# flanglet/kanzi-cpp

Measured on AMD Instinct MI355X. Metric: encode+decode MB/s on the synthetic stand-in for silesia.tar (bit-exact), higher is better.
Workload: dtype u8

## Files before the change

### kanzi-cpp_amd/csrc/bwt_fwd.hip

```cpp
#include "common.hpp"
#include "stages.hpp"
#include "bwt_common.hpp"

#include <cstdlib>
#include <cstring>
#include <algorithm>
#include <cmath>
#include "prims.hpp"
#include <chrono>
#include <vector>

namespace knz {

constexpr u32 SM_TS = 1792;
constexpr u32 SM_WIN = 2048;
constexpr u32 SM_G = 256;
constexpr u32 MED_CAP = 8192;
constexpr u32 SUPER_CAP = 8192;
constexpr int GATHER_THREADS = 512;
constexpr u32 GATHER_ROWS = 16;
static_assert(MED_CAP <= GATHER_ROWS * GATHER_THREADS, "k_bwt_f_gather_desc judges a medium group from one batch of loads");
constexpr u32 LARGE_OS_MIN = 1000000;
constexpr u32 NO_BIT = 0x7FFFFFFFu;

struct FwdView {
    const u32* base;
    int nBlocks;
    u32 total;
    u32* SA;
    u32* ISA;
    u64* ISA2;
    u32 round;
    u32* K;
    u32* gbits;
    u32* gnew;
    u32* counters;
    const u32* ovr;
    const u32* rtbits;
    uint2* medStage;
};

enum FwdCounter : u32 {
    CNT_SMALL_LEFT = 0,
    CNT_MED = 1,
    CNT_LARGE = 2,
    CNT_LARGE_MEMBERS = 3,
    CNT_RUN = 4,
    CNT_RUN_MEMBERS = 5,
    CNT_RUN_LONGEST = 6,
    CNT_SUPER = 7,
    CNT_RUNS = 8,
    CNT_STAT_SMALL = 10,
    CNT_STAT_SMALL_GROUPS = 11,
    CNT_STAT_MED = 12,
    CNT_TIED = 13,
    CNT_PROBE_CAND = 14,
    CNT_LINKED = 14,
    CNT_LINK_TIED = 15,
    CNT_STAT_MED_GROUPS = 16,
    CNT_STAT_UNSPLIT = 17,
    CNT_STAT_UNSPLIT_MEMBERS = 18,
    CNT_STAT_MAJ = 19,
    CNT_STAT_MAJ_MEMBERS = 20,
    CNT_ROUND_SLOTS = 24,
    CNT_PROBE_SLOTS = 2,
    CNT_LONGEST_BLOCK = 32,
    CNT_NSYM = 33,
};

constexpr u32 LAB_BITS = 28;
constexpr u64 LAB_MASK = (1ull << LAB_BITS) - 1ull;

__device__ __forceinline__ u32 lab_old(const FwdView& v, u32 q, u32 bb)
{
    if (v.ISA2 == nullptr) return v.ISA[q];
    const u64 e = v.ISA2[q];
    const u32 rel = ((u32)(e >> 56) == v.round && v.round != 0) ? (u32)((e >> LAB_BITS) & LAB_MASK) : (u32)(e & LAB_MASK);
    return bb + rel;
}
__device__ __forceinline__ u32 lab_cur(const FwdView& v, u32 q, u32 bb)
{
    if (v.ISA2 == nullptr) return v.ISA[q];
    return bb + (u32)(v.ISA2[q] & LAB_MASK);
}
__device__ __forceinline__ void lab_set(const FwdView& v, u32 p, u32 bb, u32 lab, u32 was)
{
    if (v.ISA2 == nullptr) { v.ISA[p] = lab; return; }
#ifdef KNZ_EMU
    if (v.round != 0 && lab_old(v, p, bb) != was) {
        fprintf(stderr, "lab_set: round %u position %u: was %u, label %u\n", v.round, p, was, lab_old(v, p, bb));
        abort();
    }
#endif
    const u64 nw = (u64)(lab - bb), ow = (v.round == 0) ? nw : (u64)(was - bb);
    v.ISA2[p] = nw | (ow << LAB_BITS) | ((u64)v.round << 56);
}

__device__ __forceinline__ u32 gather_key(const FwdView& v, u32 gp, u32 h, u32 blkBase, u32 blkEnd)
{
    const u32 q = gp + h;
    return (q < blkEnd) ? lab_old(v, q, blkBase) - blkBase + 1u : 0u;
}

__device__ __forceinline__ void classify_child(const FwdView& v, uint2* __restrict__ medNext, uint2* __restrict__ largeNext, u32 start, u32 size, u32& surv)
{
    if (size > MED_CAP) {
        const u32 at = atomicAdd(&v.counters[CNT_LARGE], 1u);
        largeNext[at] = make_uint2(start, size);
        atomicAdd(&v.counters[CNT_LARGE_MEMBERS], size);
    } else if (size > SM_G) {
        v.medStage[start >> 8] = make_uint2(start, size);
    } else if (size > 1) {
        surv = 1;
    }
}

struct ClassAgg { u32 cnt[3]; u32 elems[3]; u32 base[3]; };

__device__ __forceinline__ void agg_init(ClassAgg& A) { if (threadIdx.x < 3) { A.cnt[threadIdx.x] = 0; A.elems[threadIdx.x] = 0; A.base[threadIdx.x] = 0; } }

__device__ __forceinline__ int agg_note(ClassAgg& A, u32 size, bool run, u32& surv, u32& local)
{
    int kind;
    if (run) kind = 2;
    else if (size > MED_CAP) kind = 1;
    else if (size > SM_G) kind = 0;
    else { if (size > 1) surv = 1; return -1; }
    if (kind != 0) { local = atomicAdd(&A.cnt[kind], 1u); atomicAdd(&A.elems[kind], size); }
    return kind;
}

__device__ __forceinline__ void agg_reserve(ClassAgg& A, const FwdView& v)
{
    if (A.cnt[1]) { A.base[1] = atomicAdd(&v.counters[CNT_LARGE], A.cnt[1]); atomicAdd(&v.counters[CNT_LARGE_MEMBERS], A.elems[1]); }
    if (A.cnt[2]) { A.base[2] = atomicAdd(&v.counters[CNT_RUN], A.cnt[2]); atomicAdd(&v.counters[CNT_RUN_MEMBERS], A.elems[2]); }
}

__device__ __forceinline__ void agg_write(const ClassAgg& A, const FwdView& v, int kind, u32 local, u32 start, u32 size, uint2* __restrict__ largeNext,
                                          uint2* __restrict__ runList)
{
    if (kind == 0) { v.medStage[start >> 8] = make_uint2(start, size); return; }
    uint2* dst = kind == 1 ? largeNext : runList;
    dst[A.base[kind] + local] = make_uint2(start, size);
}

__global__ void k_bwt_bases(BwtView v, u32* __restrict__ base, u8* __restrict__ ok, u32* __restrict__ maxLen, int suffixOnly)
// ... 674 lines not shown
}

__device__ __forceinline__ u32 link_next_zero(const u32* __restrict__ posflag, const u32* __restrict__ sufRev, u32 nW, u32 p)
{
    const u32 w = p >> 5;
    const u32 x = ~posflag[w] & (0xFFFFFFFFu << (p & 31));
    if (x) return 32u * w + (u32)__ffs((int)x) - 1u;
    return (w + 1 < nW) ? sufRev[nW - 2 - w] : 0xFFFFFFFFu;
}

__global__ __launch_bounds__(256) void k_bwt_f_link_apply(FwdView v, const u32* __restrict__ posflag, const u32* __restrict__ sufRev, u32 nW,
                                                          const u32* __restrict__ linked, u32 h, u32* __restrict__ ovr, u32* __restrict__ rtbits, u32 tileStep, LinkTrial tr)
{
    __shared__ SmWindow W;
    __shared__ int sAny;
    __shared__ u32 sLinked[64];
    __shared__ u32 sRt[64];
    __shared__ u32 sOff[SM_WIN];
    u32 tile, posLo, posHi;
    if (!link_tile(v, tr, tileStep, tile, posLo, posHi)) return;
    const u32 slot0 = tile * SM_TS;
    if (threadIdx.x >= 64 && threadIdx.x < 128) { sLinked[threadIdx.x - 64] = linked[(slot0 >> 5) + threadIdx.x - 64]; sRt[threadIdx.x - 64] = 0; }
    if (!sm_load_window(v, slot0, W, &sAny)) return;
    __syncthreads();
    u32 gs[SM_WIN / 256], ge[SM_WIN / 256];
    bool act[SM_WIN / 256];
#pragma unroll
    for (int k = 0; k < (int)(SM_WIN / 256); k++) {
        const u32 i = threadIdx.x + 256u * k;
        act[k] = sm_group_of(W, i, gs[k], ge[k]) && ((sLinked[gs[k] >> 5] >> (gs[k] & 31)) & 1u);
        if (act[k] && i == gs[k]) {
            const u32 gp = v.SA[slot0 + i];
            const u32 e = link_next_zero(posflag, sufRev, nW, gp);
            sOff[i] = (e != 0xFFFFFFFFu && e > gp) ? (e - gp) + h : 0u;
        }
    }
    __syncthreads();
#pragma unroll
    for (int k = 0; k < (int)(SM_WIN / 256); k++) {
        if (!act[k]) continue;
        const u32 i = threadIdx.x + 256u * k;
        const u32 off = sOff[gs[k]];
        if (off == 0) continue;
        const u32 slot = slot0 + i;
        const bool had = (rtbits[slot >> 5] >> (slot & 31)) & 1u;
        const u32 old = had ? ovr[slot] : 0u;
        if (off > old) ovr[slot] = off;
        if (!had) atomicOr(&sRt[i >> 5], 1u << (i & 31));
    }
    __syncthreads();
    if (threadIdx.x < 64 && sRt[threadIdx.x]) atomicOr(&rtbits[(slot0 >> 5) + threadIdx.x], sRt[threadIdx.x]);
}

template <int ROWS>
__device__ __forceinline__ bool gather_rows(const FwdView& v, u32 gs, u32 n, u32 off, u32 bb, u32 be, bool judge, u32 key0, u32* sDiff)
{
    u32 gp[ROWS], key[ROWS];
#pragma unroll
    for (int k = 0; k < ROWS; k++) { const u32 i = (u32)k * GATHER_THREADS + threadIdx.x; gp[k] = (i < n) ? v.SA[gs + i] : bb; }
#pragma unroll
    for (int k = 0; k < ROWS; k++) { const u32 i = (u32)k * GATHER_THREADS + threadIdx.x; key[k] = (i < n) ? gather_key(v, gp[k], off, bb, be) : key0; }
    if (judge) {
        bool diff = false;
#pragma unroll
        for (int k = 0; k < ROWS; k++) diff = diff || key[k] != key0;
        if (__ballot(diff) != 0 && (threadIdx.x & 63) == 0) *sDiff = 1;
        __syncthreads();
        if (*sDiff == 0) return true;
    }
#pragma unroll
    for (int k = 0; k < ROWS; k++) { const u32 i = (u32)k * GATHER_THREADS + threadIdx.x; if (i < n) v.K[gs + i] = key[k]; }
    return false;
}

__global__ __launch_bounds__(GATHER_THREADS) void k_bwt_f_gather_desc(FwdView v, uint2* __restrict__ desc, u32 nDesc, u32 h, uint2* __restrict__ descInfo, int stats, int skip)
{
    __shared__ int sBlk;
    __shared__ u32 sDiff;
    const u32 xcd = blockIdx.x & 7, lanesPerXcd = gridDim.x >> 3, slot = blockIdx.x >> 3;
    const u32 per = (nDesc + 7) / 8;
    const u32 lo = xcd * per, hi = (lo + per < nDesc) ? lo + per : nDesc;
    for (u32 g = lo + slot; g < hi; g += lanesPerXcd) {
        const uint2 d = desc[g];
        if (threadIdx.x == 0) { sBlk = find_block(v.base, v.nBlocks, d.x); sDiff = 0; }
        __syncthreads();
        const u32 bb = v.base[sBlk], be = v.base[sBlk + 1];
        u32 off = h;
        if (v.rtbits && ((v.rtbits[d.x >> 5] >> (d.x & 31)) & 1u)) { const u32 r = v.ovr[d.x]; off = r > h ? r : h; }
        const u32 gp0 = v.SA[d.x];
        const u32 lab = lab_old(v, gp0, bb), key0 = gather_key(v, gp0, off, bb, be);
        const bool judge = skip && d.y > SM_G && d.y <= GATHER_ROWS * (u32)GATHER_THREADS && lab - d.x < d.y;
        bool unsplit = false;
        if (d.y <= 1 * GATHER_THREADS) unsplit = gather_rows<1>(v, d.x, d.y, off, bb, be, judge, key0, &sDiff);
        else if (d.y <= 2 * GATHER_THREADS) unsplit = gather_rows<2>(v, d.x, d.y, off, bb, be, judge, key0, &sDiff);
        else if (d.y <= 4 * GATHER_THREADS) unsplit = gather_rows<4>(v, d.x, d.y, off, bb, be, judge, key0, &sDiff);
        else if (d.y <= 8 * GATHER_THREADS) unsplit = gather_rows<8>(v, d.x, d.y, off, bb, be, judge, key0, &sDiff);
        else for (u32 i0 = 0; i0 < d.y; i0 += GATHER_ROWS * GATHER_THREADS)
            unsplit = gather_rows<(int)GATHER_ROWS>(v, d.x + i0, d.y - i0, off, bb, be, judge, key0, &sDiff);
        if (threadIdx.x == 0) {
            descInfo[g] = make_uint2(bb, lab);
            if (unsplit) { v.medStage[d.x >> 8] = d; desc[g] = make_uint2(d.x, 0u); }
            if (stats && d.y) {
                atomicAdd(&v.counters[CNT_STAT_MED], d.y); atomicAdd(&v.counters[CNT_STAT_MED_GROUPS], 1u);
                if (unsplit) { atomicAdd(&v.counters[CNT_STAT_UNSPLIT], 1u); atomicAdd(&v.counters[CNT_STAT_UNSPLIT_MEMBERS], d.y); }
            }
        }
        __syncthreads();
    }
}

template <int THREADS, int ROWS>
struct MedLds {
    static constexpr int WAVES = THREADS / 64;
    static constexpr u32 CAP = (u32)ROWS * THREADS;
    u32 oK[CAP];
    u32 oV[CAP];
    u32 cnt[WAVES * 256];
    u32 fb[CAP / 32];
    int pm[CAP / 32];
    u32 pn[CAP / 32];
    u32 wtot[WAVES];
    u32 wtot2[WAVES];
    u32 oldLab;
    u32 blkBase;
};

template <int THREADS, int ROWS>
__device__ __forceinline__ u32 med_block_sum(MedLds<THREADS, ROWS>& L, u32 x)
{
    const u32 s = wave_sum(x);
    if ((threadIdx.x & 63) == 0) L.wtot[threadIdx.x >> 6] = s;
    __syncthreads();
    u32 tot = 0;
    for (int w = 0; w < THREADS / 64; w++) tot += L.wtot[w];
    __syncthreads();
    return tot;
}

template <int THREADS, int ROWS>
__device__ __forceinline__ void med_radix_sort(MedLds<THREADS, ROWS>& L, u32 n, int npass)
{
    constexpr int WAVES = THREADS / 64;
    const int tid = (int)threadIdx.x, lane = tid & 63, wave = tid >> 6;
    const unsigned long long ltMask = (lane == 0) ? 0ull : (~0ull >> (64 - lane));
    u32* cntw = L.cnt + wave * 256;
    const int R = (int)((n + THREADS - 1) / THREADS);
    const u32 waveBase = (u32)wave * (u32)R * 64u;
    for (int pass = 0; pass < npass; pass++) {
        const int shift = 8 * pass;
        for (int q = lane; q < 256; q += 64) cntw[q] = 0;
        u32 key[ROWS], val[ROWS], pre[ROWS];
#pragma unroll
        for (int r = 0; r < ROWS; r++) {
            key[r] = 0xFFFFFFFFu; val[r] = 0; pre[r] = 0;
            if (r < R) {
                const u32 idx = waveBase + (u32)r * 64u + (u32)lane;
                if (idx < n) { key[r] = L.oK[idx]; val[r] = L.oV[idx]; }
                const u32 dg = (key[r] >> shift) & 255u;
                const unsigned long long peers = prims::digit_peers_fast(true, dg);
                const u32 pop = (u32)__popcll(peers);
                const u32 rnk = (u32)__popcll(peers & ltMask);
                const int leader = __ffsll((long long)peers) - 1;
                u32 old = 0;
                if (lane == leader) { old = cntw[dg]; cntw[dg] = old + pop; }
                old = (u32)__shfl((int)old, leader, 64);
                pre[r] = old + rnk;
            }
        }
        __syncthreads();
        {
            constexpr int TPD = THREADS / 256;
            const int dg = tid / TPD, w0 = (tid % TPD) * 4;
            const u32 c0 = L.cnt[(w0 + 0) * 256 + dg], c1 = L.cnt[(w0 + 1) * 256 + dg], c2 = L.cnt[(w0 + 2) * 256 + dg], c3 = L.cnt[(w0 + 3) * 256 + dg];
            const u32 sum = c0 + c1 + c2 + c3;
            const u32 incl = wave_incl_scan(sum);
            if (lane == 63) L.wtot[wave] = incl;
            __syncthreads();
            u32 wbase = 0;
            for (int w = 0; w < wave; w++) wbase += L.wtot[w];
            const u32 excl = wbase + incl - sum;
            L.cnt[(w0 + 0) * 256 + dg] = excl;
            L.cnt[(w0 + 1) * 256 + dg] = excl + c0;
            L.cnt[(w0 + 2) * 256 + dg] = excl + c0 + c1;
            L.cnt[(w0 + 3) * 256 + dg] = excl + c0 + c1 + c2;
        }
        __syncthreads();
#pragma unroll
        for (int r = 0; r < ROWS; r++) {
            if (r < R) {
                const u32 dg = (key[r] >> shift) & 255u;
// ... 882 lines not shown
        for (int which = 0; which < 2; which++) {
            const unsigned long long mask = which ? rm : hm;
            u32* dst = which ? rtbits : v.gnew;
            if (mask == 0) continue;
            const u32 p0 = (u32)(mask << sh);
            const u32 p1 = sh ? (u32)(mask >> (32 - sh)) : (u32)(mask >> 32);
            const u32 p2 = sh ? (u32)(mask >> (64 - sh)) : 0u;
            if (p0) atomicOr(&dst[w0], p0);
            if (p1) atomicOr(&dst[w0 + 1], p1);
            if (p2) atomicOr(&dst[w0 + 2], p2);
        }
    }
}

__global__ __launch_bounds__(256) void k_bwt_f_merge_bits(u32* __restrict__ gbits, u32* __restrict__ gnew, u32 nWords)
{
    const u32 w = blockIdx.x * 256 + threadIdx.x;
    if (w >= nWords) return;
    const u32 x = gnew[w];
    if (x) { gbits[w] |= x; gnew[w] = 0; }
}

__global__ __launch_bounds__(256) void k_bwt_f_emit(BwtView v, const u32* __restrict__ base, const u8* __restrict__ ok, const u32* __restrict__ SA,
                                                    FwdView fv, u32* __restrict__ newLen)
{
    const int b = blockIdx.y;
    if (!ok[b]) return;
    const u32 n = v.len[b];
    u32 pIndexSize = 0;
    bwt_fwd_applies(n, v.cap[b], &pIndexSize);
    const int chunks = bwt_chunks(n);
    const u32 hdr = 1 + (u32)chunks * pIndexSize;
    const u8* s = v.src[b];
    u8* d = v.dst[b];
    const u32 bb = base[b];
    const u32 r0 = lab_cur(fv, bb, bb) - bb;
    const u32 qLo = hdr + 1, qHi = hdr + n;
    const bool al = (reinterpret_cast<uintptr_t>(d) & 3) == 0;
    for (u32 w = (qLo >> 2) + blockIdx.x * 256 + threadIdx.x; 4 * w < qHi; w += gridDim.x * 256) {
        u32 word = 0, have = 0;
#pragma unroll
        for (u32 k = 0; k < 4; k++) {
            const u32 q = 4 * w + k;
            if (q >= qLo && q < qHi) {
                const u32 rr = q - qLo;
                const u32 r = rr + (rr >= r0 ? 1u : 0u);
                const u32 p = SA[bb + r] - bb;
                word |= (u32)s[p - 1] << (8 * k);
                have |= 1u << k;
            }
        }
        if (have == 0xF && al) reinterpret_cast<u32*>(d)[w] = word;
        else for (u32 k = 0; k < 4; k++) if ((have >> k) & 1) d[4 * w + k] = (u8)(word >> (8 * k));
    }
    if (blockIdx.x == 0 && threadIdx.x == 0) {
        d[hdr] = s[n - 1];
        const u32 st = n / (u32)chunks;
        const u32 step = ((u32)chunks * st == n) ? st : st + 1;
        const u32 logNbChunks = (u32)ilog2_u32((u32)chunks);
        d[0] = (u8)((logNbChunks << 2) | (pIndexSize - 1));
        u32 idx = 1;
        for (int k = 0; k < chunks; k++) {
            const u32 prim = lab_cur(fv, bb + (u32)k * step, bb) - bb;
            for (int sh = (int)(pIndexSize - 1) * 8; sh >= 0; sh -= 8) d[idx++] = (u8)(prim >> sh);
        }
        newLen[b] = hdr + n;
    }
}

__global__ __launch_bounds__(256) void k_bwt_f_med_flags(const uint2* __restrict__ stage, u32 nSlots, u32* __restrict__ flags)
{
    const u32 i = blockIdx.x * 256 + threadIdx.x;
    if (i < nSlots) flags[i] = stage[i].y ? 1u : 0u;
}

__global__ __launch_bounds__(256) void k_bwt_f_med_compact(uint2* __restrict__ stage, u32 nSlots, const u32* __restrict__ prefix, uint2* __restrict__ medNext)
{
    const u32 i = blockIdx.x * 256 + threadIdx.x;
    if (i >= nSlots) return;
    const uint2 d = stage[i];
    if (d.y) { medNext[prefix[i]] = d; stage[i] = make_uint2(0u, 0u); }
}

struct FwdTuning { int nsym; int noRunRound; int runFallback; int stats; int link; int plainLabels; int noPack; int noUnsplitSkip; };
static FwdTuning& fwd_tuning()
{
    static FwdTuning t = [] {
        FwdTuning x; x.nsym = 0; x.noRunRound = 0; x.runFallback = 0; x.stats = 0; x.link = 1; x.plainLabels = 0; x.noPack = 0; x.noUnsplitSkip = 0;
        if (getenv("KNZ_BWT_PLAIN_LABELS")) x.plainLabels = 1;
        if (getenv("KNZ_BWT_NO_PACK")) x.noPack = 1;
        if (getenv("KNZ_BWT_NO_UNSPLIT_SKIP")) x.noUnsplitSkip = 1;
        if (const char* e = getenv("KNZ_BWT_LINK")) x.link = atoi(e);
        if (getenv("KNZ_BWT_STATS")) x.stats = 1;
        if (const char* e = getenv("KNZ_BWT_NSYM")) x.nsym = atoi(e);
        if (getenv("KNZ_BWT_NO_RUN_ROUND")) x.noRunRound = 1;
        if (getenv("KNZ_BWT_RUN_FALLBACK")) x.runFallback = 1;
        return x;
    }();
    return t;
}
int bwt_forward_tune(const char* key, int value)
{
    FwdTuning& t = fwd_tuning();
    if (!strcmp(key, "rs_onesweep")) { prims::rs_onesweep_knob().store(value); return 0; }
    if (!strcmp(key, "bwt_nsym")) t.nsym = value;
    else if (!strcmp(key, "bwt_no_run_round")) t.noRunRound = value;
    else if (!strcmp(key, "bwt_run_fallback")) t.runFallback = value;
    else if (!strcmp(key, "bwt_stats")) t.stats = value;
    else if (!strcmp(key, "bwt_link")) t.link = value;
    else if (!strcmp(key, "bwt_plain_labels")) t.plainLabels = value;
    else if (!strcmp(key, "bwt_no_pack")) t.noPack = value;
    else if (!strcmp(key, "bwt_no_unsplit_skip")) t.noUnsplitSkip = value;
    else return -1;
    return 0;
}

struct FwdScratch {
    u64* keysA; u64* keysB;
    u32* valsA; u32* valsB;
    u32* SA; u32* ISA; u32* K; u64* ISA2;
    u32* t0; u32* t1; u32* t2; u32* t3;
    u32* gbits; u32* gnew; u32* rtbits; u32* ovr; size_t gbitsWords;
    uint2* med[2]; uint2* medStage; u32* medFlags; u32* medPrefix; size_t medSlots; uint2* descInfo; uint2* large[2]; uint2* runList; uint4* superList; u32* ebits;
    u32* loff; u32* lbase;
    u32* survTile;
    u32* linkedTile;
    u32* base;
    u32* counters;
    u32* seg2;
    void* scanTmp;
    void* rsMem;
    u32* byteHist;
    u32* classTab; u32* rbits; u32* rcount; u32* rprefix;
    u32* runPos; u32* runE; u32* runL; u32* sE; u32* rcnt; u32* moff;
    u64* runKeysA; u64* runKeysB; u64* sKey;
    size_t maxRuns;
};

static size_t fwd_align(size_t x) { return (x + 255) & ~(size_t)255; }

static size_t fwd_carve(u8* p, int nBlocks, size_t total, FwdScratch* w, u32 VS)
{
    u8* q = p;
    auto take = [&](size_t sz) { u8* r = q; q += fwd_align(sz); return r; };
    const size_t maxMed = 2 * (total / (SM_G + 1) + 2), maxLarge = total / (MED_CAP + 1) + 2;
    w->gbitsWords = ((total + 64) / 64 + SM_WIN / 64 + 4) * 2 + 128;
    w->keysA = (u64*)take(8 * total); w->keysB = (u64*)take(8 * total);
    w->valsA = (u32*)take(4 * total); w->valsB = (u32*)take(4 * total);
    w->SA = (u32*)take(4 * total); w->ISA = (u32*)take(4 * total); w->K = (u32*)take(4 * total);
    w->ISA2 = (VS <= (1u << LAB_BITS)) ? (u64*)take(8 * total) : (u64*)nullptr;
    w->t0 = (u32*)take(4 * total); w->t1 = (u32*)take(4 * total); w->t2 = (u32*)take(4 * total); w->t3 = (u32*)take(4 * total);
    w->gbits = (u32*)take(4 * w->gbitsWords);
    w->gnew = (u32*)take(4 * w->gbitsWords);
    w->rtbits = (u32*)take(4 * w->gbitsWords);
    w->ovr = (u32*)take(4 * total);
    w->med[0] = (uint2*)take(8 * maxMed); w->med[1] = (uint2*)take(8 * maxMed);
    w->medSlots = total / 256 + 2;
    w->medStage = (uint2*)take(8 * w->medSlots); w->medFlags = (u32*)take(4 * w->medSlots + 64); w->medPrefix = (u32*)take(4 * w->medSlots + 64);
    w->large[0] = (uint2*)take(8 * maxLarge); w->large[1] = (uint2*)take(8 * maxLarge);
    w->runList = (uint2*)take(8 * maxMed);
    w->superList = (uint4*)take(16 * maxMed);
    w->descInfo = (uint2*)take(8 * maxMed);
    w->ebits = (u32*)take(4 * w->gbitsWords);
    w->loff = (u32*)take(4 * (maxMed + 1));
    w->lbase = (u32*)take(4 * (maxMed + 1));
    w->survTile = (u32*)take(4 * (total / SM_TS + 64));
    w->linkedTile = (u32*)take(4 * (total / SM_TS + 64));
    w->base = (u32*)take(4ull * (nBlocks + 2));
    w->counters = (u32*)take(256);
    w->byteHist = (u32*)take(1024ull * (nBlocks + 1));
    w->seg2 = (u32*)take(64);
    w->scanTmp = take(prims::scan_tmp_bytes(total + 16));
    w->rsMem = take(prims::rs_ws_bytes(total, nBlocks + 1));
    w->maxRuns = total / 4 + 64;
    w->classTab = (u32*)take(1024ull * (size_t)nBlocks);
    const size_t rw = total / 32 + SM_WIN / 32 + 136;
    w->rbits = (u32*)take(4 * rw); w->rcount = (u32*)take(4 * rw); w->rprefix = (u32*)take(4 * rw);
    w->runPos = (u32*)take(4 * w->maxRuns); w->runE = (u32*)take(4 * w->maxRuns); w->runL = (u32*)take(4 * w->maxRuns);
    w->sE = (u32*)take(4 * w->maxRuns); w->rcnt = (u32*)take(4 * w->maxRuns); w->moff = (u32*)take(4 * w->maxRuns + 64);
    w->runKeysA = (u64*)take(8 * w->maxRuns); w->runKeysB = (u64*)take(8 * w->maxRuns); w->sKey = (u64*)take(8 * w->maxRuns);
    return (size_t)(q - p);
}

size_t bwt_forward_scratch_bytes(int nBlocks, u32 VS, size_t total)
{
    FwdScratch w;
    return fwd_carve(nullptr, nBlocks, total, &w, VS) + 4096;
}

#define GRID1(n) dim3((unsigned)(((n) + 255) / 256)), dim3(256), 0, s

static int bits_for(u64 n, int lo) { while ((1ull << lo) < n) lo++; return lo; }

struct LinkPlan {
    enum Mode { UNTRIED, TRIAL, ON, APPLIED, OFF } mode = UNTRIED;
    int trials = 0; u32 retryH = 0xFFFFFFFFu;
    bool next(u32 h, u32 survMembers, u32 total, u32 linked, u32 tied, bool stats)
    {
        if (mode == TRIAL || mode == APPLIED) {
            const bool paid = linked >= 4096 && tied < linked / 2;
            mode = paid ? ON : OFF;
            if (!paid) retryH = (trials < 2) ? h * 8 : 0xFFFFFFFFu;
            if (stats) fprintf(stderr, "link step: %u members linked, %u of the windows' members still tied after the round -> %s\n", linked, tied, paid ? "on" : "off");
        }
        if (mode == OFF && h >= retryH) mode = UNTRIED;
        if (mode == UNTRIED && survMembers >= total / 8) { mode = TRIAL; trials++; return true; }
        if (mode == ON && survMembers >= total / 64) { mode = APPLIED; return true; }
        return false;
    }
};

struct FwdSort {
    hipStream_t s; const XfStage& st; u32* hp;
    const FwdTuning tune = fwd_tuning();
    BwtView bv; FwdView v; FwdScratch w; size_t maxTotal;
    prims::RsWs rs1;
    u32 total, medSlots, nTiles; int nsym, pbits, kbits;
    u32 h = 1; int cur = 0;
    u64 *keysFree, *keysFree2;
    u32 nRun, runElems, surv, nMed, nLarge, largeElems, survMembers;
    LinkPlan link; LinkTrial linkTr; std::chrono::steady_clock::time_point statT;
    int fetch(u32 first, u32 n) { return hipMemcpyAsync(hp + first, w.counters + first, 4 * (size_t)n, hipMemcpyDeviceToHost, s) == hipSuccess && hipStreamSynchronize(s) == hipSuccess ? 0 : -1; }
    void merge_bits() { hipLaunchKernelGGL(k_bwt_f_merge_bits, GRID1(total / 32 + 2), w.gbits, w.gnew, total / 32 + 2); }
    void enable_run_tiebits() { if (!v.rtbits) { hipMemsetAsync(w.rtbits, 0, 4 * w.gbitsWords, s); v.ovr = w.ovr; v.rtbits = w.rtbits; } }
    void compact_medium(uint2* dst)
    {
        KScope ks_("k_bwt_f_med_compact");
        hipLaunchKernelGGL(k_bwt_f_med_flags, GRID1(medSlots), w.medStage, medSlots, w.medFlags);
        prims::launch_scan<prims::SCAN_SUM_EXCL>(s, w.medFlags, w.medPrefix, medSlots, nullptr, w.scanTmp, w.counters + CNT_MED);
        hipLaunchKernelGGL(k_bwt_f_med_compact, GRID1(medSlots), w.medStage, medSlots, w.medPrefix, dst);
    }
    void bounds(u32 n, bool last, const u32* bits = nullptr, u32 len = 0, u32 wordsPerWin = 0)
    {
        if (bits) { KScope ks_("k_bwt_f_r0_winsum"); hipLaunchKernelGGL(k_bwt_f_r0_winsum, GRID1(n), bits, len, n, w.t0, w.t2, wordsPerWin); }
        if (last) { KScope ks_("k_bwt_f_scan_max"); prims::launch_scan<prims::SCAN_MAX_INCL>(s, w.t0, w.t1, n, nullptr, w.scanTmp); }
        KScope ks_("k_bwt_f_scan_min"); prims::launch_scan<prims::SCAN_MIN_INCL>(s, w.t2, w.t3, n, nullptr, w.scanTmp);
    }
    template <class KEY, bool HAS_VAL> int sort_one_segment(u32 n, KEY* ka, KEY* kb, u32* va, u32* vb, int loBit, int hiBit, bool oneRead = true)
    {
        hipLaunchKernelGGL(prims::k_rs_one_segment, dim3(1), dim3(64), 0, s, w.seg2, n);
        prims::rs_launch_layout(s, rs1);
        return prims::rs_sort<KEY, HAS_VAL>(s, rs1, ka, kb, va, vb, (size_t)n, loBit, hiBit, oneRead);
    }
    int setup(void* scratch, size_t scratchBytes, BwtSuffixArrays* sa)
    {
        bv.src = st.src; bv.dst = st.dst; bv.len = st.len; bv.cap = st.cap; bv.VS = st.maxLen; bv.nBlocks = st.nBlocks;
        maxTotal = (size_t)st.nBlocks * bv.VS;
        if (fwd_carve(reinterpret_cast<u8*>(scratch), st.nBlocks, maxTotal, &w, bv.VS) > scratchBytes) return -2;
        { KScope ks_("k_bwt_f_bases"); hipLaunchKernelGGL(k_bwt_bases, dim3(1), dim3(64), 0, s, bv, w.base, st.ok, w.counters + CNT_LONGEST_BLOCK, sa ? 1 : 0); }
        hipMemsetAsync(st.newLen, 0, sizeof(u32) * st.nBlocks, s);
        { KScope ks_("k_bwt_f_r0_hist");
          hipMemsetAsync(w.byteHist, 0, 1024ull * st.nBlocks, s);
          hipLaunchKernelGGL(k_bwt_f_bytehist, dim3(64, (unsigned)st.nBlocks), dim3(256), 0, s, bv, w.base, w.byteHist);
          hipLaunchKernelGGL(k_bwt_f_choose_nsym, dim3(1), dim3(256), 0, s, w.byteHist, st.nBlocks, w.counters + CNT_LONGEST_BLOCK, w.counters + CNT_NSYM); }
        if (hipMemcpyAsync(hp, w.base + st.nBlocks, 4, hipMemcpyDeviceToHost, s) != hipSuccess || fetch(CNT_LONGEST_BLOCK, 2)) return -1;
        total = hp[0];
        if (sa) { sa->SA = w.SA; sa->base = w.base; sa->total = total; }
        if (total == 0) return 0;
        v.base = w.base; v.nBlocks = st.nBlocks; v.total = total; v.SA = w.SA; v.ISA = w.ISA; v.K = w.K; v.ISA2 = (w.ISA2 != nullptr && !tune.plainLabels) ? w.ISA2 : (u64*)nullptr;
        v.round = 0; v.gbits = w.gbits; v.gnew = w.gnew; v.counters = w.counters; v.medStage = w.medStage; v.ovr = nullptr; v.rtbits = nullptr;
        medSlots = (u32)((size_t)total / 256 + 1); nTiles = (total + SM_TS - 1) / SM_TS;
        survMembers = total;
        hipMemsetAsync(w.medStage, 0, 8ull * w.medSlots, s);
        pbits = bits_for(hp[CNT_LONGEST_BLOCK], 1);
        const int fit = (64 - pbits) / 8, want = (hp[CNT_NSYM] == 5u) ? 5 : 4;
        nsym = fit < want ? fit : want;
        if (tune.nsym >= 1) nsym = tune.nsym < fit ? tune.nsym : fit;
        if (nsym < 1) return -4;
        while (2 * h <= (u32)nsym) h <<= 1;
        return 0;
    }
    void round0_sort()
    {
        const prims::RsWs rs = prims::rs_carve(w.rsMem, maxTotal, st.nBlocks + 1, w.base, st.nBlocks);
        rs1 = prims::rs_carve(w.rsMem, maxTotal, st.nBlocks + 1, w.seg2, 1);
        { KScope ks_("k_bwt_f_r0_layout"); prims::rs_launch_layout(s, rs); }
        u64* kin = w.keysA; u64* kout = w.keysB;
        const bool oneRead = prims::rs_onesweep_knob().load() != 0 && nsym <= prims::RS_MAXPASS
                             && (size_t)bv.VS < (size_t)prims::RS_VAL_MASK;
        if (oneRead) {
            KScope ks_("k_bwt_f_r0_sort");
            hipLaunchKernelGGL(k_bwt_f_r0_counts, dim3((unsigned)rs.L.nSeg), dim3(256), 0, s, bv, w.base, w.byteHist, nsym, rs.L);
            hipLaunchKernelGGL(prims::k_rs_digit_bases, dim3((unsigned)rs.L.nSeg, (unsigned)nsym), dim3(256), 0, s, rs.L);
        }
        auto sortPass = [&](const auto& src, int pass) {
            if (oneRead) prims::rs_launch_pass_os<u64, false>(s, rs, src, nullptr, kout, nullptr, (size_t)bv.VS, pass);
            else prims::rs_launch_pass<u64, false>(s, rs, src, nullptr, kout, nullptr, (size_t)bv.VS);
        };
        for (int pass = 0; pass < nsym; pass++) {
            KScope ks_("k_bwt_f_r0_sort");
            if (pass == 0) { TextSrc src; src.src = bv.src; src.P = nsym; src.pbits = pbits; src.shift = pbits; sortPass(src, pass); }
            else { prims::DigitOfKey<u64> src; src.keys = kin; src.shift = pbits + 8 * pass; src.mask = 255u; sortPass(src, pass); }
            std::swap(kin, kout);
        }
        keysFree = kout; keysFree2 = kin;
    }
    int round0_place()
    {
        hipMemsetAsync(w.gbits, 0xFF, 4 * w.gbitsWords, s); hipMemsetAsync(w.gnew, 0, 4 * w.gbitsWords, s);
        hipMemsetAsync(w.counters, 0, 4 * CNT_ROUND_SLOTS, s);
        { KScope ks_("k_bwt_f_r0_flags"); hipLaunchKernelGGL(k_bwt_f_r0_flags, dim3((total + 256 * R0F_ROWS - 1) / (256 * R0F_ROWS)), dim3(256), 0, s, keysFree2, w.base, st.nBlocks, total, nsym, pbits,
                                                             reinterpret_cast<unsigned long long*>(w.gbits)); }
        bounds(nTiles, true, w.gbits, total, SM_TS / 32);
        kbits = bits_for((u64)bv.VS + 2, 1);
        const bool runRound = (2 * kbits + 1) < 64 && !tune.noRunRound;
        { KScope ks_("k_bwt_f_r0_place");
          hipLaunchKernelGGL(k_bwt_f_r0_place_text, dim3(nTiles), dim3(256), 0, s, bv, v, w.t1, w.t3, nTiles, w.large[cur], keysFree2, nsym, pbits, runRound ? w.runList : (uint2*)nullptr);
          merge_bits(); }
        if (fetch(0, CNT_ROUND_SLOTS)) return -1;
        nRun = hp[CNT_RUN]; runElems = hp[CNT_RUN_MEMBERS];
        return 0;
    }
    int run_fallback()
    {
        { KScope ks_("k_bwt_f_run_fallback"); hipLaunchKernelGGL(k_bwt_f_run_fallback, GRID1(nRun), v, w.runList, nRun, w.med[cur], w.large[cur]); }
        nRun = 0; return fetch(0, CNT_ROUND_SLOTS);
    }
    int run_round()
    {
        if (nRun && ((u64)nRun > (1ull << (64 - (2 * kbits + 1))) || tune.runFallback) && run_fallback()) return -1;
        if (!nRun) return 0;
        const u32 nWin = (total + SM_WIN - 1) / SM_WIN;
        { KScope ks_("k_bwt_f_run_ends"); hipLaunchKernelGGL(k_bwt_f_run_ends, dim3(nWin), dim3(256), 0, s, bv, v, reinterpret_cast<u8*>(w.ebits)); }
        bounds(nWin, false, w.ebits, total, SM_WIN / 32);
        hipMemsetAsync(w.classTab, 0xFF, 1024ull * (size_t)st.nBlocks, s);
        { KScope ks_("k_bwt_f_run_classes"); hipLaunchKernelGGL(k_bwt_f_run_classes, GRID1(nRun), bv, v, w.runList, nRun, w.classTab); }
        { KScope ks_("k_bwt_f_run_len"); hipLaunchKernelGGL(k_bwt_f_run_len, dim3(nWin), dim3(256), 0, s, bv, v, w.ebits, w.t3, nWin, w.K, w.classTab, (u32)nsym,
                                                            reinterpret_cast<unsigned long long*>(w.rbits), w.rcount); }
        const u32 nRW = nWin * (SM_WIN / 32);
        { KScope ks_("k_bwt_f_scan_sum"); prims::launch_scan<prims::SCAN_SUM_EXCL>(s, w.rcount, w.rprefix, nRW, nullptr, w.scanTmp, w.counters + CNT_RUNS); }
        { KScope ks_("k_bwt_f_run_compact"); hipLaunchKernelGGL(k_bwt_f_run_compact, GRID1(nRW), w.rbits, w.rprefix, nRW, w.runPos); }
        if (fetch(CNT_RUN_LONGEST, 3)) return -1;
        const u32 nRuns = hp[CNT_RUNS];
        const int hbits = bits_for((u64)hp[CNT_RUN_LONGEST] + 1, 1) + 1;
        const int rbits = bits_for(nRun, 0), idxBits = bits_for(nRuns, 1);
        if (nRuns == 0 || nRuns > w.maxRuns || rbits + hbits > 32 || idxBits + kbits + 1 + rbits > 64) return run_fallback();
        { KScope ks_("k_bwt_f_large_prefix"); hipLaunchKernelGGL(k_bwt_f_large_prefix, dim3(1), dim3(1024), 0, s, w.runList, nRun, w.loff, w.base, st.nBlocks, w.lbase); }
        { KScope ks_("k_bwt_f_run_table"); hipLaunchKernelGGL(k_bwt_f_run_table, GRID1(nRuns), bv, v, w.runPos, nRuns, w.K, w.classTab, kbits, idxBits, w.runKeysA, w.runE, w.runL); }
        const u64* rkSorted;
        { KScope ks_("k_bwt_f_sort_runs");
          rkSorted = sort_one_segment<u64, false>(nRuns, w.runKeysA, w.runKeysB, nullptr, nullptr, idxBits, idxBits + kbits + 1 + rbits) ? w.runKeysB : w.runKeysA; }
        { KScope ks_("k_bwt_f_run_sorted"); hipLaunchKernelGGL(k_bwt_f_run_sorted, GRID1(nRuns), rkSorted, nRuns, idxBits, w.runE, w.runL, (u32)nsym, w.sE, w.sKey, w.rcnt); }
        { KScope ks_("k_bwt_f_scan_sum"); prims::launch_scan<prims::SCAN_SUM_EXCL>(s, w.rcnt, w.moff, nRuns, nullptr, w.scanTmp); }
        { KScope ks_("k_bwt_f_run_members"); hipLaunchKernelGGL(k_bwt_f_run_members, dim3((runElems + 2047) / 2048), dim3(256), 0, s, w.moff, nRuns, runElems, w.sKey, kbits, hbits,
                                                                (u32)nsym, keysFree); }
        u64* rk; u32* rv = w.valsA;
// ... 24 lines not shown
            hipMemsetAsync(w.counters, 0, 4 * CNT_PROBE_SLOTS, s);
            { KScope ks_("k_bwt_f_probe");
              hipLaunchKernelGGL(k_bwt_f_probe, dim3(std::min<u32>(nCand, 4096)), dim3(512), 0, s, bv, v, w.med[cur], probeCand, nCand, (u32)nsym, w.med[cur ^ 1], w.large[cur], w.ovr, w.rtbits);
              merge_bits(); }
            compact_medium(w.med[cur] + nMed);
            if (fetch(0, CNT_PROBE_SLOTS)) return -1;
            surv |= hp[CNT_SMALL_LEFT]; nMed += hp[CNT_MED];
        }
        if (tune.stats) fprintf(stderr, "after round 0 (nsym %d, total %u): run groups %u (%u members); small left %u, medium %u, large %u (%u members)\n",
                                nsym, total, nRun, runElems, surv, nMed, nLarge, largeElems);
        statT = std::chrono::steady_clock::now();
        return 0;
    }
    void link_step()
    {
        KScope ks_("k_bwt_f_link");
        u32* posflag = w.ebits; u32* linked = w.rbits; u32* rev = w.rcount; u32* sufRev = w.rprefix;
        const bool trial = link.mode == LinkPlan::TRIAL; linkTr.n = 0;
        if (trial) { linkTr.blk[linkTr.n++] = 0; if (st.nBlocks >= 5) linkTr.blk[linkTr.n++] = st.nBlocks / 2; if (st.nBlocks >= 3) linkTr.blk[linkTr.n++] = st.nBlocks - 1; }
        const u32 nW = total / 32 + 1;
        hipMemsetAsync(posflag, 0, 4 * (size_t)nW, s);
        hipMemsetAsync(linked, 0, 4 * ((size_t)nTiles * (SM_TS / 32) + 64), s);
        enable_run_tiebits();
        const u32 nTrial = (u32)std::min<u64>((u64)nTiles, ((u64)bv.VS + SM_TS - 1) / SM_TS + 2);
        const dim3 gridL(trial ? nTrial : nTiles, (unsigned)(linkTr.n ? linkTr.n : 1));
        hipLaunchKernelGGL(k_bwt_f_link_small, gridL, dim3(256), 0, s, v, posflag, linked, tune.stats, 1u, w.linkedTile, linkTr);
        hipLaunchKernelGGL(k_bwt_f_link_zeros, GRID1(nW), posflag, nW, rev);
        prims::launch_scan<prims::SCAN_MIN_INCL>(s, rev, sufRev, nW, nullptr, w.scanTmp);
        hipLaunchKernelGGL(k_bwt_f_link_apply, gridL, dim3(256), 0, s, v, posflag, sufRev, nW, linked, h, w.ovr, w.rtbits, 1u, linkTr);
    }
    void sort_small(bool linked)
    {
        KScope ks_("k_bwt_f_sort_small");
        u32* survTile = tune.link ? w.survTile : nullptr;
        if (v.ISA2 && pbits <= 23 && !tune.noPack) hipLaunchKernelGGL(k_bwt_f_small_fused<true>, dim3(nTiles), dim3(256), 0, s, v, h, survTile, tune.stats);
        else if (v.ISA2) hipLaunchKernelGGL(k_bwt_f_small_fused<false>, dim3(nTiles), dim3(256), 0, s, v, h, survTile, tune.stats);
        else hipLaunchKernelGGL(k_bwt_f_sort_small, dim3(nTiles), dim3(256), 0, s, v, survTile);
        if (linked) hipLaunchKernelGGL(k_bwt_f_link_payoff, dim3(1), dim3(256), 0, s, v, w.linkedTile, w.survTile, nTiles, 1u, w.counters + CNT_LINKED, linkTr);
        if (tune.link) prims::launch_scan<prims::SCAN_SUM_EXCL>(s, w.survTile, w.survTile, nTiles, nullptr, w.scanTmp, w.counters + CNT_TIED);
    }
    void sort_medium()
    {
        const int npass = (kbits + 7) / 8, nxt = cur ^ 1;
        { KScope ks_("k_bwt_f_sort_medium"); const dim3 gridM(std::min<u32>(nMed, 8192));
          const auto sort256 = tune.stats ? k_bwt_f_sort_medium<256, 8, true> : k_bwt_f_sort_medium<256, 8, false>;
          const auto sort512 = tune.stats ? k_bwt_f_sort_medium<512, 16, true> : k_bwt_f_sort_medium<512, 16, false>;
          hipLaunchKernelGGL(sort256, gridM, dim3(256), 0, s, v, w.med[cur], nMed, npass, SM_G, w.med[nxt], w.large[nxt], w.descInfo, w.superList);
          hipLaunchKernelGGL(sort512, gridM, dim3(512), 0, s, v, w.med[cur], nMed, npass, 2048u, w.med[nxt], w.large[nxt], w.descInfo, w.superList); }
        { KScope ks_("k_bwt_f_super"); hipLaunchKernelGGL(k_bwt_f_super, dim3(std::min<u32>(nMed, 512)), dim3(1024), 0, s, v, w.superList, h, npass, w.med[nxt], w.large[nxt]); }
    }
    template <class KEY> void large_keys()
    {
        { KScope ks_("k_bwt_f_large_prefix"); hipLaunchKernelGGL(k_bwt_f_large_prefix, dim3(1), dim3(1024), 0, s, w.large[cur], nLarge, w.loff, w.base, st.nBlocks, w.lbase); }
        KScope ks_("k_bwt_f_large_keys");
        hipLaunchKernelGGL(k_bwt_f_large_keys<KEY>, GRID1(largeElems), v, w.large[cur], nLarge, w.loff, largeElems, h, kbits, reinterpret_cast<KEY*>(keysFree), w.valsA);
    }
    template <class KEY> void sort_large(int lbits)
    {
        KEY* ka = reinterpret_cast<KEY*>(keysFree); KEY* kb = reinterpret_cast<KEY*>(keysFree2); int r;
        { KScope ks_("k_bwt_f_sort_large");
          r = sort_one_segment<KEY, true>(largeElems, ka, kb, w.valsA, w.valsB, 0, kbits + lbits, largeElems >= LARGE_OS_MIN); }
        const KEY* sk = r ? kb : ka; const u32* sv = r ? w.valsB : w.valsA;
        { KScope ks_("k_bwt_f_large_flags"); hipLaunchKernelGGL(k_bwt_f_large_flags<KEY>, GRID1(largeElems), sk, largeElems, w.t0, w.t2); }
        bounds(largeElems, true);
        { KScope ks_("k_bwt_f_large_place");
          hipLaunchKernelGGL(k_bwt_f_large_place<KEY>, GRID1(largeElems), v, w.large[cur], w.loff, largeElems, kbits, sk, sv, w.t1, w.t3, w.med[cur ^ 1], w.large[cur ^ 1], w.lbase); }
    }
    int end_round()
    {
        { KScope ks_("k_bwt_f_merge_bits"); merge_bits(); }
        compact_medium(w.med[cur ^ 1]);
        if (fetch(0, CNT_ROUND_SLOTS)) return -1;
        surv = hp[CNT_SMALL_LEFT]; nMed = hp[CNT_MED]; nLarge = hp[CNT_LARGE]; largeElems = hp[CNT_LARGE_MEMBERS]; survMembers = hp[CNT_TIED];
        if (tune.stats) {
            std::vector<u32> hs(nTiles); u32 activeTiles = 0;
            if (tune.link && hipMemcpyAsync(hs.data(), w.survTile, 4 * (size_t)nTiles, hipMemcpyDeviceToHost, s) == hipSuccess && hipStreamSynchronize(s) == hipSuccess) {
                for (u32 t = 0; t + 1 < nTiles; t++) activeTiles += hs[t + 1] != hs[t] ? 1u : 0u;
                fprintf(stderr, "  windows with tied small groups after the round: %u of %u\n", activeTiles, nTiles);
            }
            const std::chrono::steady_clock::time_point now = std::chrono::steady_clock::now();
            fprintf(stderr, "round h=%u (%.3f ms): small members worked on %u in %u groups, medium members %u; after it: small left %u, medium groups %u, large %u (%u members); %u groups took the chain round; %u small members still tied\n",
                    h, std::chrono::duration<double, std::milli>(now - statT).count(), hp[CNT_STAT_SMALL], hp[CNT_STAT_SMALL_GROUPS], hp[CNT_STAT_MED], surv, nMed, nLarge, largeElems,
                    hp[CNT_SUPER], hp[CNT_TIED]);
            fprintf(stderr, "  medium groups worked on %u (%u members): all keys equal in %u (%u members)%s, majority path %u (%u members)\n", hp[CNT_STAT_MED_GROUPS], hp[CNT_STAT_MED],
                    hp[CNT_STAT_UNSPLIT], hp[CNT_STAT_UNSPLIT_MEMBERS], tune.noUnsplitSkip ? "" : " -- left alone", hp[CNT_STAT_MAJ], hp[CNT_STAT_MAJ_MEMBERS]);
            statT = now;
        }
        cur ^= 1; h <<= 1;
        return 0;
    }
    int round()
    {
        if (h > bv.VS) return -5;
        { KScope ks_("k_bwt_f_round"); hipMemsetAsync(w.counters, 0, 4 * CNT_ROUND_SLOTS, s); }
        if (++v.round > 255) return -5;
        const bool linked = surv && tune.link && h >= (u32)(tune.link > 1 ? tune.link : 32)
                            && link.next(h, survMembers, total, hp[CNT_LINKED], hp[CNT_LINK_TIED], tune.stats);
        if (linked) link_step();
        if (surv && !v.ISA2) { KScope ks_("k_bwt_f_gather_small"); hipLaunchKernelGGL(k_bwt_f_gather_small, dim3(nTiles), dim3(256), 0, s, v, h, tune.stats); }
        if (nMed) { KScope ks_("k_bwt_f_gather_desc"); hipLaunchKernelGGL(k_bwt_f_gather_desc, dim3(1024), dim3(GATHER_THREADS), 0, s, v, w.med[cur], nMed, h, w.descInfo, tune.stats, tune.noUnsplitSkip ? 0 : 1); }
        const int lbits = bits_for(nLarge, 0); const bool key32 = kbits + lbits <= 32;
        if (nLarge) { if (key32) large_keys<u32>(); else large_keys<u64>(); }
        if (surv) sort_small(linked);
        if (nMed) sort_medium();
        if (nLarge) { if (key32) sort_large<u32>(lbits); else sort_large<u64>(lbits); }
        return end_round();
    }
    void emit()
    {
        KScope ks_("k_bwt_f_emit");
        hipLaunchKernelGGL(k_bwt_f_emit, dim3((unsigned)std::min<size_t>(((size_t)bv.VS + 255) / 256, 4096), st.nBlocks), dim3(256), 0, s, bv, w.base, st.ok, w.SA, v, st.newLen);
    }
};

static int bwt_forward_run(hipStream_t s, const XfStage& st, void* scratch, size_t scratchBytes, u32* h_pinned, BwtSuffixArrays* sa)
{
    FwdSort f{ s, st, h_pinned };
    if (int r = f.setup(scratch, scratchBytes, sa)) return r;
    if (f.total == 0) return 0;
    f.round0_sort();
    if (f.round0_place() || f.run_round() || f.probe()) return -1;
    while (f.surv || f.nMed || f.nLarge) if (int r = f.round()) return r;
    if (!sa) f.emit();
    return hipGetLastError() == hipSuccess ? 0 : -1;
}

int launch_bwt_forward(hipStream_t s, const XfStage& st, void* scratch, size_t scratchBytes, u32* h_pinned)
{ return bwt_forward_run(s, st, scratch, scratchBytes, h_pinned, nullptr); }
int bwt_suffix_arrays(hipStream_t s, const XfStage& st, void* scratch, size_t scratchBytes, u32* h_pinned, BwtSuffixArrays* out)
{ return bwt_forward_run(s, st, scratch, scratchBytes, h_pinned, out); }

}
```

Measured before the change: 6405.

## Put unsplit medium BWT groups to sleep using previous-round verdicts

Records a per-group verdict (round, status, size, key) when a medium group's gather finds all keys equal. A new pre-pass kernel then checks whether a group that was unsplit last round points, through a chain of two other unsplit groups, to a state that guarantees it stays unsplit. If so, it marks the group as skipped before the gather kernel runs, so the group avoids a full key gather. This adds a verdict buffer, a binary-search kernel launch each round, and correctness risk if the inference is wrong for some inputs.

```diff
diff --git a/kanzi-cpp_amd/csrc/bwt_fwd.hip b/kanzi-cpp_amd/csrc/bwt_fwd.hip
--- a/kanzi-cpp_amd/csrc/bwt_fwd.hip
+++ b/kanzi-cpp_amd/csrc/bwt_fwd.hip
@@ -38,7 +38,13 @@
     const u32* ovr;
     const u32* rtbits;
     uint2* medStage;
+    uint2* verdictNow;
+    const uint2* verdictWas;
 };
+
+constexpr u32 VERDICT_WHOLE = 1, VERDICT_PLAIN = 2;
+__host__ __device__ __forceinline__ u32 verdict_word(u32 round, u32 status, u32 members) { return (round << 24) | (status << 16) | members; }
+static_assert(MED_CAP < (1u << 16), "verdict_word keeps a medium group's size in 16 bits");
 
 enum FwdCounter : u32 {
     CNT_SMALL_LEFT = 0,
@@ -62,6 +68,8 @@
     CNT_STAT_UNSPLIT_MEMBERS = 18,
     CNT_STAT_MAJ = 19,
     CNT_STAT_MAJ_MEMBERS = 20,
+    CNT_STAT_ASLEEP = 21,
+    CNT_STAT_ASLEEP_MEMBERS = 22,
     CNT_ROUND_SLOTS = 24,
     CNT_PROBE_SLOTS = 2,
     CNT_LONGEST_BLOCK = 32,
@@ -902,6 +910,7 @@
     const u32 lo = xcd * per, hi = (lo + per < nDesc) ? lo + per : nDesc;
     for (u32 g = lo + slot; g < hi; g += lanesPerXcd) {
         const uint2 d = desc[g];
+        if (d.y == 0) continue;
         if (threadIdx.x == 0) { sBlk = find_block(v.base, v.nBlocks, d.x); sDiff = 0; }
         __syncthreads();
         const u32 bb = v.base[sBlk], be = v.base[sBlk + 1];
@@ -919,13 +928,52 @@
             unsplit = gather_rows<(int)GATHER_ROWS>(v, d.x + i0, d.y - i0, off, bb, be, judge, key0, &sDiff);
         if (threadIdx.x == 0) {
             descInfo[g] = make_uint2(bb, lab);
-            if (unsplit) { v.medStage[d.x >> 8] = d; desc[g] = make_uint2(d.x, 0u); }
-            if (stats && d.y) {
+            if (unsplit) {
+                v.medStage[d.x >> 8] = d; desc[g] = make_uint2(d.x, 0u);
+                if (v.verdictNow) v.verdictNow[d.x >> 8] = make_uint2(key0, verdict_word(v.round, (off == h && key0 != 0u) ? VERDICT_PLAIN : VERDICT_WHOLE, d.y));
+            }
+            if (stats) {
                 atomicAdd(&v.counters[CNT_STAT_MED], d.y); atomicAdd(&v.counters[CNT_STAT_MED_GROUPS], 1u);
                 if (unsplit) { atomicAdd(&v.counters[CNT_STAT_UNSPLIT], 1u); atomicAdd(&v.counters[CNT_STAT_UNSPLIT_MEMBERS], d.y); }
             }
         }
         __syncthreads();
+    }
+}
+
+__device__ __forceinline__ bool sleep_target(const FwdView& v, const uint2* __restrict__ desc, u32 nDesc, u32 lab, u32 bb, bool plain, u32& start, u32& key)
+{
+    u32 lo = 0, hi = nDesc;
+    while (lo < hi) { const u32 mid = (lo + hi) >> 1; if (desc[mid].x <= lab) lo = mid + 1; else hi = mid; }
+    if (lo == 0) return false;
+    start = desc[lo - 1].x;
+    const uint2 t = v.verdictWas[start >> 8];
+    const u32 status = (t.y >> 16) & 3u;
+    if ((t.y >> 24) != v.round - 1u || (plain ? status != VERDICT_PLAIN : status == 0u) || lab - start >= (t.y & 0xFFFFu)) return false;
+    key = t.x;
+    return lab_old(v, v.SA[start], bb) == lab;
+}
+
+__global__ __launch_bounds__(256) void k_bwt_f_med_sleep(FwdView v, uint2* __restrict__ desc, u32 nDesc, int stats)
+{
+    const u32 g = blockIdx.x * 256 + threadIdx.x;
+    if (g >= nDesc) return;
+    const uint2 d = desc[g];
+    if (d.y <= SM_G || d.y > MED_CAP) return;
+    const uint2 was = v.verdictWas[d.x >> 8];
+    if (was.y != verdict_word(v.round - 1u, VERDICT_PLAIN, d.y)) return;
+    if (v.rtbits && ((v.rtbits[d.x >> 5] >> (d.x & 31)) & 1u)) return;
+    const u32 bb = v.base[find_block(v.base, v.nBlocks, d.x)];
+    u32 s1, k1, s2, k2;
+    if (!sleep_target(v, desc, nDesc, bb + was.x - 1u, bb, true, s1, k1) || s1 == d.x) return;
+    if (!sleep_target(v, desc, nDesc, bb + k1 - 1u, bb, false, s2, k2) || s2 == d.x) return;
+    v.verdictNow[d.x >> 8] = make_uint2(k1, verdict_word(v.round, VERDICT_PLAIN, d.y));
+    v.medStage[d.x >> 8] = d;
+    desc[g] = make_uint2(d.x, 0u);
+    if (stats) {
+        atomicAdd(&v.counters[CNT_STAT_MED], d.y); atomicAdd(&v.counters[CNT_STAT_MED_GROUPS], 1u);
+        atomicAdd(&v.counters[CNT_STAT_UNSPLIT], 1u); atomicAdd(&v.counters[CNT_STAT_UNSPLIT_MEMBERS], d.y);
+        atomicAdd(&v.counters[CNT_STAT_ASLEEP], 1u); atomicAdd(&v.counters[CNT_STAT_ASLEEP_MEMBERS], d.y);
     }
 }
 
@@ -1974,14 +2022,15 @@
     if (d.y) { medNext[prefix[i]] = d; stage[i] = make_uint2(0u, 0u); }
 }
 
-struct FwdTuning { int nsym; int noRunRound; int runFallback; int stats; int link; int plainLabels; int noPack; int noUnsplitSkip; };
+struct FwdTuning { int nsym; int noRunRound; int runFallback; int stats; int link; int plainLabels; int noPack; int noUnsplitSkip; int noGroupSleep; };
 static FwdTuning& fwd_tuning()
 {
     static FwdTuning t = [] {
-        FwdTuning x; x.nsym = 0; x.noRunRound = 0; x.runFallback = 0; x.stats = 0; x.link = 1; x.plainLabels = 0; x.noPack = 0; x.noUnsplitSkip = 0;
+        FwdTuning x; x.nsym = 0; x.noRunRound = 0; x.runFallback = 0; x.stats = 0; x.link = 1; x.plainLabels = 0; x.noPack = 0; x.noUnsplitSkip = 0; x.noGroupSleep = 0;
         if (getenv("KNZ_BWT_PLAIN_LABELS")) x.plainLabels = 1;
         if (getenv("KNZ_BWT_NO_PACK")) x.noPack = 1;
         if (getenv("KNZ_BWT_NO_UNSPLIT_SKIP")) x.noUnsplitSkip = 1;
+        if (getenv("KNZ_BWT_NO_GROUP_SLEEP")) x.noGroupSleep = 1;
         if (const char* e = getenv("KNZ_BWT_LINK")) x.link = atoi(e);
         if (getenv("KNZ_BWT_STATS")) x.stats = 1;
         if (const char* e = getenv("KNZ_BWT_NSYM")) x.nsym = atoi(e);
@@ -2003,6 +2052,7 @@
     else if (!strcmp(key, "bwt_plain_labels")) t.plainLabels = value;
     else if (!strcmp(key, "bwt_no_pack")) t.noPack = value;
     else if (!strcmp(key, "bwt_no_unsplit_skip")) t.noUnsplitSkip = value;
+    else if (!strcmp(key, "bwt_no_group_sleep")) t.noGroupSleep = value;
     else return -1;
     return 0;
 }
@@ -2013,7 +2063,7 @@
     u32* SA; u32* ISA; u32* K; u64* ISA2;
     u32* t0; u32* t1; u32* t2; u32* t3;
     u32* gbits; u32* gnew; u32* rtbits; u32* ovr; size_t gbitsWords;
-    uint2* med[2]; uint2* medStage; u32* medFlags; u32* medPrefix; size_t medSlots; uint2* descInfo; uint2* large[2]; uint2* runList; uint4* superList; u32* ebits;
+    uint2* med[2]; uint2* medStage; uint2* medVerdict[2]; u32* medFlags; u32* medPrefix; size_t medSlots; uint2* descInfo; uint2* large[2]; uint2* runList; uint4* superList; u32* ebits;
     u32* loff; u32* lbase;
     u32* survTile;
     u32* linkedTile;
@@ -2049,6 +2099,7 @@
     w->med[0] = (uint2*)take(8 * maxMed); w->med[1] = (uint2*)take(8 * maxMed);
     w->medSlots = total / 256 + 2;
     w->medStage = (uint2*)take(8 * w->medSlots); w->medFlags = (u32*)take(4 * w->medSlots + 64); w->medPrefix = (u32*)take(4 * w->medSlots + 64);
+    w->medVerdict[0] = (uint2*)take(16 * w->medSlots); w->medVerdict[1] = w->medVerdict[0] + w->medSlots;
     w->large[0] = (uint2*)take(8 * maxLarge); w->large[1] = (uint2*)take(8 * maxLarge);
     w->runList = (uint2*)take(8 * maxMed);
     w->superList = (uint4*)take(16 * maxMed);
@@ -2108,6 +2159,7 @@
     BwtView bv; FwdView v; FwdScratch w; size_t maxTotal;
     prims::RsWs rs1;
     u32 total, medSlots, nTiles; int nsym, pbits, kbits;
+    bool groupSleep = false;
     u32 h = 1; int cur = 0;
     u64 *keysFree, *keysFree2;
     u32 nRun, runElems, surv, nMed, nLarge, largeElems, survMembers;
@@ -2151,9 +2203,12 @@
         if (total == 0) return 0;
         v.base = w.base; v.nBlocks = st.nBlocks; v.total = total; v.SA = w.SA; v.ISA = w.ISA; v.K = w.K; v.ISA2 = (w.ISA2 != nullptr && !tune.plainLabels) ? w.ISA2 : (u64*)nullptr;
         v.round = 0; v.gbits = w.gbits; v.gnew = w.gnew; v.counters = w.counters; v.medStage = w.medStage; v.ovr = nullptr; v.rtbits = nullptr;
+        v.verdictNow = nullptr; v.verdictWas = nullptr;
         medSlots = (u32)((size_t)total / 256 + 1); nTiles = (total + SM_TS - 1) / SM_TS;
         survMembers = total;
         hipMemsetAsync(w.medStage, 0, 8ull * w.medSlots, s);
+        groupSleep = !tune.noUnsplitSkip && !tune.noGroupSleep;
+        if (groupSleep) hipMemsetAsync(w.medVerdict[0], 0, 16ull * w.medSlots, s);
         pbits = bits_for(hp[CNT_LONGEST_BLOCK], 1);
         const int fit = (64 - pbits) / 8, want = (hp[CNT_NSYM] == 5u) ? 5 : 4;
         nsym = fit < want ? fit : want;
@@ -2344,8 +2399,8 @@
             fprintf(stderr, "round h=%u (%.3f ms): small members worked on %u in %u groups, medium members %u; after it: small left %u, medium groups %u, large %u (%u members); %u groups took the chain round; %u small members still tied\n",
                     h, std::chrono::duration<double, std::milli>(now - statT).count(), hp[CNT_STAT_SMALL], hp[CNT_STAT_SMALL_GROUPS], hp[CNT_STAT_MED], surv, nMed, nLarge, largeElems,
                     hp[CNT_SUPER], hp[CNT_TIED]);
-            fprintf(stderr, "  medium groups worked on %u (%u members): all keys equal in %u (%u members)%s, majority path %u (%u members)\n", hp[CNT_STAT_MED_GROUPS], hp[CNT_STAT_MED],
-                    hp[CNT_STAT_UNSPLIT], hp[CNT_STAT_UNSPLIT_MEMBERS], tune.noUnsplitSkip ? "" : " -- left alone", hp[CNT_STAT_MAJ], hp[CNT_STAT_MAJ_MEMBERS]);
+            fprintf(stderr, "  medium groups worked on %u (%u members): all keys equal in %u (%u members)%s, majority path %u (%u members), asleep %u (%u members)\n", hp[CNT_STAT_MED_GROUPS], hp[CNT_STAT_MED],
+                    hp[CNT_STAT_UNSPLIT], hp[CNT_STAT_UNSPLIT_MEMBERS], tune.noUnsplitSkip ? "" : " -- left alone", hp[CNT_STAT_MAJ], hp[CNT_STAT_MAJ_MEMBERS], hp[CNT_STAT_ASLEEP], hp[CNT_STAT_ASLEEP_MEMBERS]);
             statT = now;
         }
         cur ^= 1; h <<= 1;
@@ -2360,6 +2415,8 @@
                             && link.next(h, survMembers, total, hp[CNT_LINKED], hp[CNT_LINK_TIED], tune.stats);
         if (linked) link_step();
         if (surv && !v.ISA2) { KScope ks_("k_bwt_f_gather_small"); hipLaunchKernelGGL(k_bwt_f_gather_small, dim3(nTiles), dim3(256), 0, s, v, h, tune.stats); }
+        if (groupSleep) { v.verdictNow = w.medVerdict[v.round & 1]; v.verdictWas = w.medVerdict[(v.round & 1) ^ 1]; }
+        if (groupSleep && nMed && v.round >= 2) { KScope ks_("k_bwt_f_med_sleep"); hipLaunchKernelGGL(k_bwt_f_med_sleep, GRID1(nMed), v, w.med[cur], nMed, tune.stats); }
         if (nMed) { KScope ks_("k_bwt_f_gather_desc"); hipLaunchKernelGGL(k_bwt_f_gather_desc, dim3(1024), dim3(GATHER_THREADS), 0, s, v, w.med[cur], nMed, h, w.descInfo, tune.stats, tune.noUnsplitSkip ? 0 : 1); }
         const int lbits = bits_for(nLarge, 0); const bool key32 = kbits + lbits <= 32;
         if (nLarge) { if (key32) large_keys<u32>(); else large_keys<u64>(); }
```

Measured after the change: 6518, median of 6. +1.8%, better.
